# llm-d/llm-d-workload-variant-autoscaler

Hardware: AMD Instinct MI355X
Metric: desired-replica accuracy + SLO-attainment %, Llama-3-8B synthetic QPS ramp (higher is better)
Workload: dtype bf16; 1 GPU; model=meta-llama/Llama-3.1-8B, global_batch=256, seq_len=150, parallelism=dp1, device=AMD Radeon Graphics

## Files before the change

### wva_amd/calibration/model.py

```python
from __future__ import annotations

import math
from dataclasses import dataclass
from typing import List, Optional

import torch

from .. import ops


@dataclass
class LlamaConfig:
    name: str = "llama"
    hidden_size: int = 4096
    intermediate_size: int = 14336
    num_layers: int = 32
    num_q_heads: int = 32
    num_kv_heads: int = 8
    head_dim: int = 128
    vocab_size: int = 128256
    rope_theta: float = 500000.0
    rms_eps: float = 1e-5

    @property
# ... 66 lines not shown
            return torch.empty(rows, cols, device=device, dtype=dtype).normal_(
                0.0, std, generator=gen
            )

        self.input_norm = torch.ones(h, device=device, dtype=dtype)
        self.post_attn_norm = torch.ones(h, device=device, dtype=dtype)
        self.wqkv = w(cfg.q_size + 2 * cfg.kv_size, h)
        self.wo = w(h, cfg.q_size)
        self.w_gate_up = w(2 * cfg.intermediate_size, h)
        self.w_down = w(h, cfg.intermediate_size)


class LlamaDecodeModel:

    def __init__(
        self,
        cfg: LlamaConfig,
        max_batch: int = 256,
        max_seq: int = 2048,
        device: str = "cuda",
        seed: int = 0,
        kv_dtype: str = "bf16",
        weights_dtype: str = "bf16",
    ):
        self.cfg = cfg
        self.device = torch.device(device)
        self.dtype = torch.bfloat16
        if weights_dtype not in ("bf16", "fp8"):
            raise ValueError(f"weights_dtype must be bf16|fp8")
        self.weights_dtype = weights_dtype
        if kv_dtype not in ("bf16", "fp8"):
            raise ValueError(f"kv_dtype must be bf16|fp8, got {kv_dtype}")
        self.kv_dtype = kv_dtype
        self.cache_dtype = (
            torch.float8_e4m3fn if kv_dtype == "fp8" else torch.bfloat16
        )
        self.max_batch = max_batch
        self.max_seq = max_seq
        gen = torch.Generator(device=self.device)
        gen.manual_seed(seed)

        self.embed = torch.empty(
            cfg.vocab_size, cfg.hidden_size, device=self.device, dtype=self.dtype
        ).normal_(0.0, 0.02, generator=gen)
        self.layers: List[_DecoderLayer] = [
            _DecoderLayer(cfg, self.device, self.dtype, gen)
            for _ in range(cfg.num_layers)
        ]
# ... 42 lines not shown
    def _linear(self, x: torch.Tensor, layer, name: str) -> torch.Tensor:
        if self.weights_dtype == "bf16":
            w = getattr(layer, name) if layer is not None else self.lm_head
            return ops.linear(x, w)
        w8, w_scale = (
            getattr(layer, name + "_q") if layer is not None else self.lm_head_q
        )
        if not x.is_cuda:
            return (
                x.float() @ (w8.float() * w_scale[:, None]).t()
            ).to(x.dtype)
        if x.shape[0] <= 64 and x.shape[1] % 128 == 0:
            from .. import ops as _ops

            return _ops._require_ext().skinny_linear_fp8(x, w8, w_scale)
        return (x @ (w8.to(x.dtype) * w_scale[:, None].to(x.dtype)).t())

    @torch.no_grad()
    def decode_step(self, token_ids: torch.Tensor) -> torch.Tensor:
        cfg = self.cfg
        B = token_ids.shape[0]
        positions = self.context_lens[:B].clone()

        ctx = positions + 1
        x = self.embed.index_select(0, token_ids)
        residual: Optional[torch.Tensor] = None

        for li, layer in enumerate(self.layers):
            if residual is None:
                residual = x.clone()
                h = ops.rmsnorm(x, layer.input_norm, None, cfg.rms_eps)
            else:
                h = ops.rmsnorm(x, layer.input_norm, residual, cfg.rms_eps)

            qkv = self._linear(h, layer, "wqkv")
            q = ops.rope_append_kv(
                qkv, self.k_cache[li][:B], self.v_cache[li][:B],
                positions, cfg.num_q_heads, cfg.num_kv_heads, cfg.rope_theta,
            )

            attn = ops.gqa_decode_attn(
                q, self.k_cache[li][:B], self.v_cache[li][:B], ctx, self.scale
            )
            x = self._linear(attn.reshape(B, cfg.q_size), layer, "wo")

            h2 = ops.rmsnorm(x, layer.post_attn_norm, residual, cfg.rms_eps)
            gate_up = self._linear(h2, layer, "w_gate_up")
            act = ops.silu_mul_fused(gate_up)
            x = self._linear(act, layer, "w_down")

        final = ops.rmsnorm(x, self.final_norm, residual, cfg.rms_eps)
        logits = self._linear(final, None, "lm_head")
        self.context_lens[:B] += 1
        return logits

    @torch.no_grad()
    def prefill(self, token_ids: torch.Tensor) -> torch.Tensor:
        cfg = self.cfg
        if self.weights_dtype != "bf16":
            raise NotImplementedError(
                "prefill with fp8 weights is not implemented (the "
                "weight-only fp8 mode targets decode; prefill would "
                "dequantize every layer per pass)"
            )
        B, S = token_ids.shape
        T = B * S
# ... 83 lines not shown
```

### wva_amd/ops/__init__.py

```python
from __future__ import annotations

import glob
import importlib.util
import math
import os
from typing import Optional

import torch

_HERE = os.path.dirname(os.path.abspath(__file__))
_ext = None
_ext_error: Optional[str] = None


def _try_load_extension():
    global _ext, _ext_error
    if _ext is not None:
        return _ext
    candidates = sorted(glob.glob(os.path.join(_HERE, "_wva_ops*.so")))
    if not candidates:
        _ext_error = (
            f"HIP extension _wva_ops*.so not found in {_HERE}; build it with "
            "`python -m wva_amd.ops.build` (or __graft_entry__.build())"
        )
# ... 238 lines not shown
    return silu_mul_ref(gate_up[:, :inter], gate_up[:, inter:]).to(
        gate_up.dtype
    )


def gqa_decode_attn(
    q: torch.Tensor,
    k_cache: torch.Tensor,
    v_cache: torch.Tensor,
    context_lens: torch.Tensor,
    scale: Optional[float] = None,
) -> torch.Tensor:
    if scale is None:
        scale = 1.0 / math.sqrt(q.shape[-1])
    if q.is_cuda:
        return _require_ext().gqa_decode_attn(
            q, k_cache, v_cache, context_lens.to(torch.int32), scale
        )
    return gqa_decode_attn_ref(q, k_cache, v_cache, context_lens, scale).to(
        q.dtype
    )


def moe_route(router_logits: torch.Tensor, top_k: int):
    if router_logits.is_cuda:
        return tuple(
            _require_ext().moe_route(
                router_logits.float().contiguous(), top_k
            )
        )
    return moe_route_ref(router_logits, top_k)


def moe_gate_up_swiglu(
    x: torch.Tensor,
    w_gate_up: torch.Tensor,
    expert_offsets: torch.Tensor,
    sorted_slots: torch.Tensor,
    top_k: int,
) -> torch.Tensor:
    if x.is_cuda:
        return _require_ext().moe_gate_up_swiglu(
            x, w_gate_up, expert_offsets, sorted_slots, top_k
        )
    return moe_gate_up_swiglu_ref(
        x, w_gate_up, expert_offsets, sorted_slots, top_k
# ... 81 lines not shown
```

### wva_amd/ops/csrc/attention.hip

```cpp
#include "common.h"

#include <type_traits>

#define HEAD_DIM 128
#define MAX_G 8
#define TILE 64
#define NUM_WAVES 4
#define ROW_DW 66
#define S_ROW 65

template <bool KV_FP8>
using kv_elem_t = std::conditional_t<KV_FP8, fp8_t, bf16>;

__device__ __forceinline__ long ws_row_offset(int b, int kvh, int g, int split,
                                              int num_kv_heads, int G,
                                              int num_splits) {
  return ((((long)b * num_kv_heads + kvh) * G + g) * num_splits + split) *
         (2 + HEAD_DIM);
}

__device__ __forceinline__ long pack8_fp8(const float* v, float inv_scale) {
  unsigned int lo = 0, hi = 0;
  lo = __builtin_amdgcn_cvt_pk_fp8_f32(v[0] * inv_scale, v[1] * inv_scale,
                                       lo, false);
  lo = __builtin_amdgcn_cvt_pk_fp8_f32(v[2] * inv_scale, v[3] * inv_scale,
                                       lo, true);
  hi = __builtin_amdgcn_cvt_pk_fp8_f32(v[4] * inv_scale, v[5] * inv_scale,
                                       hi, false);
  hi = __builtin_amdgcn_cvt_pk_fp8_f32(v[6] * inv_scale, v[7] * inv_scale,
                                       hi, true);
  return (long)(((unsigned long)hi << 32) | lo);
}

struct QFrags {
  bf16x8_frag bf[4];
  long fp8[4];
  float scale;
};

template <bool KV_FP8>
__device__ __forceinline__ QFrags load_q_frags(const bf16* __restrict__ q,
                                               int b, int kvh, int G,
                                               int num_q_heads, int lane,
                                               int wave, int g, int k0,
                                               float* qmax_lds) {
  QFrags qf;
  qf.scale = 1.0f;
#pragma unroll
  for (int kk = 0; kk < 4; ++kk) qf.fp8[kk] = 0;
  float qv[4][8];
#pragma unroll
  for (int kk = 0; kk < 4; ++kk)
#pragma unroll
    for (int i = 0; i < 8; ++i) qv[kk][i] = 0.0f;
  if (g < G) {
    const bf16* qrow = q + ((long)b * num_q_heads + kvh * G + g) * HEAD_DIM;
#pragma unroll
    for (int kk = 0; kk < 4; ++kk) {
      const short* src = reinterpret_cast<const short*>(qrow + 32 * kk + k0);
#pragma unroll
      for (int i = 0; i < 8; ++i) {
        qf.bf[kk][i] = src[i];
        const bf16 bv = *reinterpret_cast<const bf16*>(&src[i]);
        qv[kk][i] = bf2f(bv);
      }
    }
  } else {
#pragma unroll
    for (int kk = 0; kk < 4; ++kk)
#pragma unroll
      for (int i = 0; i < 8; ++i) qf.bf[kk][i] = 0;
  }
  if constexpr (KV_FP8) {
    float amax = 0.0f;
#pragma unroll
    for (int kk = 0; kk < 4; ++kk)
#pragma unroll
      for (int i = 0; i < 8; ++i) amax = fmaxf(amax, fabsf(qv[kk][i]));
    amax = wave_reduce_max(amax);
    if (lane == 0) qmax_lds[wave] = amax;
    __syncthreads();
    float m0 = qmax_lds[0];
#pragma unroll
    for (int w2 = 1; w2 < NUM_WAVES; ++w2) m0 = fmaxf(m0, qmax_lds[w2]);
    qf.scale = fmaxf(m0 / 448.0f, 1e-12f);
    const float inv = 1.0f / qf.scale;
#pragma unroll
    for (int kk = 0; kk < 4; ++kk) qf.fp8[kk] = pack8_fp8(qv[kk], inv);
    __syncthreads();
  }
  return qf;
}

struct SoftmaxStep {
  float p;
  float corr;
};

__device__ __forceinline__ SoftmaxStep online_softmax_step(
    const float* __restrict__ s_row, int tn, int lane, float& m, float& s) {
  const bool live = lane < tn;
  const float score = live ? s_row[lane] : -INFINITY;
  const float tile_max = wave_reduce_max(score);
  const float m_new = fmaxf(m, tile_max);
  const float p = live ? __expf(score - m_new) : 0.0f;
  const float tile_sum = wave_reduce_sum(p);
  const float corr = (m == -INFINITY) ? 0.0f : __expf(m - m_new);
  s = s * corr + tile_sum;
  m = m_new;
  return {p, corr};
}

template <bool KV_FP8>
__global__ __launch_bounds__(256, 2) void gqa_decode_attn_v4_kernel(
    bf16* __restrict__ out,
    float* __restrict__ workspace,
    const bf16* __restrict__ q,
    const void* __restrict__ k_cache,
    const void* __restrict__ v_cache,
    const int* __restrict__ context_lens,
    const int num_q_heads,
    const int num_kv_heads,
    const int max_seq,
    const float scale) {
  const int b = blockIdx.x;
  const int kvh = blockIdx.y;
  const int split = blockIdx.z;
  const int num_splits = gridDim.z;
  const int G = num_q_heads / num_kv_heads;
  const int ctx = context_lens[b];

  const int lane = threadIdx.x & (WAVE_SIZE - 1);
  const int wave = threadIdx.x / WAVE_SIZE;
  const int frag_col = lane % 16;
  const int frag_k0 = 8 * (lane / 16);

  __shared__ float s_smem[MAX_G][S_ROW];
  __shared__ unsigned int v_smem[TILE * ROW_DW];
  __shared__ float p_smem[MAX_G][TILE];
  float* qmax_lds = nullptr;
  if constexpr (KV_FP8) {
    __shared__ float qmax_smem[NUM_WAVES];
    qmax_lds = qmax_smem;
  }

  const QFrags qf = load_q_frags<KV_FP8>(q, b, kvh, G, num_q_heads, lane,
                                         wave, frag_col, frag_k0, qmax_lds);

  const int heads_mine = (G > wave) ? (G - wave + NUM_WAVES - 1) / NUM_WAVES : 0;
  float m[2], s[2], acc[2][2];
#pragma unroll
  for (int j = 0; j < 2; ++j) {
    m[j] = -INFINITY;
    s[j] = 0.0f;
    acc[j][0] = acc[j][1] = 0.0f;
  }

  const long slab_off = ((long)b * num_kv_heads + kvh) * max_seq * HEAD_DIM;
  const auto* k_slab =
      reinterpret_cast<const kv_elem_t<KV_FP8>*>(k_cache) + slab_off;
  const auto* v_slab =
      reinterpret_cast<const kv_elem_t<KV_FP8>*>(v_cache) + slab_off;

  for (int t0 = split * TILE; t0 < ctx; t0 += num_splits * TILE) {
    const int tn = min(TILE, ctx - t0);

    if constexpr (KV_FP8) {
      const int tile_g8 = tn * (HEAD_DIM / 8);
      const fp8_t* v_src = v_slab + (long)t0 * HEAD_DIM;
      for (int idx = wave * WAVE_SIZE + lane; idx < tile_g8;
// ... 93 lines not shown
  if (num_splits == 1) {
    for (int j = 0; j < heads_mine; ++j) {
      const int g = wave + j * NUM_WAVES;
      const float inv = s[j] > 0.0f ? 1.0f / s[j] : 0.0f;
      bf16x2* orow = reinterpret_cast<bf16x2*>(
          out + ((long)b * num_q_heads + kvh * G + g) * HEAD_DIM);
      orow[lane] = bf16x2{f2bf(acc[j][0] * inv), f2bf(acc[j][1] * inv)};
    }
  } else {
    for (int j = 0; j < heads_mine; ++j) {
      const int g = wave + j * NUM_WAVES;
      float* wsp = workspace +
          ws_row_offset(b, kvh, g, split, num_kv_heads, G, num_splits);
      if (lane == 0) {
        wsp[0] = m[j];
        wsp[1] = s[j];
      }
      wsp[2 + 2 * lane] = acc[j][0];
      wsp[2 + 2 * lane + 1] = acc[j][1];
    }
  }
}

template <bool KV_FP8>
__global__ __launch_bounds__(256, 2) void gqa_decode_attn_v5_kernel(
    bf16* __restrict__ out,
    float* __restrict__ workspace,
    const bf16* __restrict__ q,
    const void* __restrict__ k_cache,
    const void* __restrict__ v_cache,
    const int* __restrict__ context_lens,
    const int num_q_heads,
    const int num_kv_heads,
    const int max_seq,
    const float scale) {
  const int b = blockIdx.x;
  const int kvh = blockIdx.y;
  const int split = blockIdx.z;
  const int num_splits = gridDim.z;
  const int G = num_q_heads / num_kv_heads;
  const int ctx = context_lens[b];

  const int lane = threadIdx.x & (WAVE_SIZE - 1);
  const int wave = threadIdx.x / WAVE_SIZE;
  const int frag_col = lane % 16;
  const int frag_k0 = 8 * (lane / 16);

  __shared__ float s_smem[MAX_G][S_ROW];
  __shared__ unsigned int v_smem[TILE * ROW_DW];
  __shared__ float p_smem[MAX_G][TILE];
  __shared__ float corr_smem[MAX_G];
  __shared__ float sum_smem[MAX_G];
  __shared__ float m_smem[MAX_G];
  float* qmax_lds = nullptr;
  if constexpr (KV_FP8) {
    __shared__ float qmax_smem[NUM_WAVES];
    qmax_lds = qmax_smem;
  }

  const QFrags qf = load_q_frags<KV_FP8>(q, b, kvh, G, num_q_heads, lane,
                                         wave, frag_col, frag_k0, qmax_lds);

  const int heads_mine = (G > wave) ? (G - wave + NUM_WAVES - 1) / NUM_WAVES : 0;
  float m[2], s[2];
#pragma unroll
  for (int j = 0; j < 2; ++j) {
    m[j] = -INFINITY;
    s[j] = 0.0f;
  }
  f32x4_frag acc_pv[2] = {f32x4_frag{0.f, 0.f, 0.f, 0.f},
                          f32x4_frag{0.f, 0.f, 0.f, 0.f}};

  const long slab_off = ((long)b * num_kv_heads + kvh) * max_seq * HEAD_DIM;
  const auto* k_slab =
      reinterpret_cast<const kv_elem_t<KV_FP8>*>(k_cache) + slab_off;
  const auto* v_slab =
      reinterpret_cast<const kv_elem_t<KV_FP8>*>(v_cache) + slab_off;

  for (int t0 = split * TILE; t0 < ctx; t0 += num_splits * TILE) {
    const int tn = min(TILE, ctx - t0);

    if constexpr (KV_FP8) {
      const int tile_g8 = tn * (HEAD_DIM / 8);
      const fp8_t* v_src = v_slab + (long)t0 * HEAD_DIM;
      for (int idx = wave * WAVE_SIZE + lane; idx < tile_g8;
           idx += NUM_WAVES * WAVE_SIZE) {
        const int row = idx >> 4;
        const int d8 = (idx & 15) * 8;
        const unsigned short* src =
            reinterpret_cast<const unsigned short*>(
                v_src + (long)row * HEAD_DIM + d8);
        unsigned int* dst = &v_smem[row * ROW_DW + d8 / 2];
#pragma unroll
        for (int j = 0; j < 4; ++j) {
          const float2_vt f = unpk2_fp8(src[j]);
          const bf16x2 packed{f2bf(f[0]), f2bf(f[1])};
          dst[j] = *reinterpret_cast<const unsigned int*>(&packed);
        }
      }
    } else {
      typedef __attribute__((ext_vector_type(2))) unsigned int uint2_t;
      const int tile_u2 = tn * (HEAD_DIM / 4);
      const unsigned int* v_src =
          reinterpret_cast<const unsigned int*>(v_slab + (long)t0 * HEAD_DIM);
      for (int idx = wave * WAVE_SIZE + lane; idx < tile_u2;
           idx += NUM_WAVES * WAVE_SIZE) {
        const int row = idx >> 5;
        const int d2 = (idx & 31) * 2;
        const uint2_t val = *reinterpret_cast<const uint2_t*>(&v_src[idx * 2]);
        *reinterpret_cast<uint2_t*>(&v_smem[row * ROW_DW + d2]) = val;
      }
    }

    {
      const int prow = 16 * wave + (lane % 16);
      const int pos = t0 + prow;
      const int pos_c = pos < max_seq ? pos : max_seq - 1;
      const int k0 = frag_k0;
      f32x4_frag sf = {0.f, 0.f, 0.f, 0.f};
      if constexpr (KV_FP8) {
        const long* ksrc = reinterpret_cast<const long*>(
            k_slab + (long)pos_c * HEAD_DIM);
        const int l0 = k0 / 8;
#pragma unroll
        for (int kk = 0; kk < 4; ++kk) {
          const long a8 = ksrc[kk * 4 + l0];
          sf = __builtin_amdgcn_mfma_f32_16x16x32_fp8_fp8(
              a8, qf.fp8[kk], sf, 0, 0, 0);
        }
      } else {
#pragma unroll
        for (int kk = 0; kk < 4; ++kk) {
          bf16x8_frag a_frag;
          const short* src = reinterpret_cast<const short*>(
              k_slab + (long)pos_c * HEAD_DIM) + 32 * kk + k0;
#pragma unroll
          for (int i = 0; i < 8; ++i) a_frag[i] = src[i];
          sf = __builtin_amdgcn_mfma_f32_16x16x32_bf16(a_frag, qf.bf[kk],
                                                       sf, 0, 0, 0);
        }
      }
      const float s_eff = KV_FP8 ? scale * qf.scale : scale;
      const int g = lane & 15;
      if (g < G) {
#pragma unroll
        for (int i = 0; i < 4; ++i) {
          const int t = 16 * wave + (lane >> 4) * 4 + i;
          s_smem[g][t] = (t < tn) ? sf[i] * s_eff : -INFINITY;
        }
      }
    }
    __syncthreads();

    for (int j = 0; j < heads_mine; ++j) {
      const int g = wave + j * NUM_WAVES;
      const SoftmaxStep st = online_softmax_step(s_smem[g], tn, lane, m[j], s[j]);
      p_smem[g][lane] = st.p;
      if (lane == 0) corr_smem[g] = st.corr;
    }
    __syncthreads();

    {
      bf16x8_frag p_frag[2];
#pragma unroll
      for (int kk = 0; kk < 2; ++kk) {
        const int g = lane % 16;
        const int pos0 = 32 * kk + 8 * (lane / 16);
        if (g < G) {
#pragma unroll
          for (int i = 0; i < 8; ++i)
            p_frag[kk][i] = f2bf_bits(p_smem[g][pos0 + i]);
        } else {
#pragma unroll
          for (int i = 0; i < 8; ++i) p_frag[kk][i] = 0;
        }
      }
      const unsigned short* v_u16 =
          reinterpret_cast<const unsigned short*>(v_smem);
#pragma unroll
      for (int nsub = 0; nsub < 2; ++nsub) {
        const int dim = 16 * (wave + 4 * nsub) + (lane % 16);
        f32x4_frag d = acc_pv[nsub];
#pragma unroll
        for (int i = 0; i < 4; ++i) {
          const int h = (lane >> 4) * 4 + i;
          d[i] *= (h < G) ? corr_smem[h] : 0.0f;
        }
#pragma unroll
        for (int kk = 0; kk < 2; ++kk) {
          bf16x8_frag v_frag;
          const int pos0 = 32 * kk + 8 * (lane / 16);
#pragma unroll
          for (int i = 0; i < 8; ++i) {
            const int t = pos0 + i;
            v_frag[i] = (t < tn)
                ? (short)v_u16[(t * ROW_DW + (dim >> 1)) * 2 + (dim & 1)]
                : (short)0;
          }
          d = __builtin_amdgcn_mfma_f32_16x16x32_bf16(p_frag[kk], v_frag, d,
                                                      0, 0, 0);
        }
        acc_pv[nsub] = d;
      }
    }
    __syncthreads();
  }

  for (int j = 0; j < heads_mine; ++j) {
    const int g = wave + j * NUM_WAVES;
    if (lane == 0) {
      sum_smem[g] = s[j];
      m_smem[g] = m[j];
    }
  }
  __syncthreads();

  if (num_splits == 1) {
#pragma unroll
    for (int nsub = 0; nsub < 2; ++nsub) {
      const int dim = 16 * (wave + 4 * nsub) + (lane & 15);
#pragma unroll
// ... 101 lines not shown
  if (max_ctx_hint > 0) {
    const int by_work = max_ctx_hint / (min_tiles * TILE);
    if (by_work > cap) cap = by_work;
  }
  if (splits > cap) splits = cap;
  const int max_useful = max_ctx_hint > 0 ? (max_ctx_hint + 2 * TILE - 1) / (2 * TILE) : splits;
  if (splits > max_useful && max_useful >= 1) splits = max_useful;
  return splits < 1 ? 1 : splits;
}

extern "C" void launch_gqa_decode_attn(
    void* out, void* workspace, const void* q, const void* k_cache,
    const void* v_cache, const int* context_lens, int batch, int num_q_heads,
    int num_kv_heads, int max_seq, int num_splits, float scale, int variant,
    int kv_fp8, hipStream_t stream) {
  const auto kernel =
      variant == 5 ? (kv_fp8 ? gqa_decode_attn_v5_kernel<true>
                             : gqa_decode_attn_v5_kernel<false>)
                   : (kv_fp8 ? gqa_decode_attn_v4_kernel<true>
                             : gqa_decode_attn_v4_kernel<false>);
  hipLaunchKernelGGL(kernel, dim3(batch, num_kv_heads, num_splits), dim3(256),
                     0, stream, (bf16*)out, (float*)workspace, (const bf16*)q,
                     k_cache, v_cache, context_lens, num_q_heads, num_kv_heads,
                     max_seq, scale);
  if (num_splits > 1) {
    hipLaunchKernelGGL(gqa_decode_attn_merge_kernel,
                       dim3(batch, num_q_heads), dim3(64 * MERGE_WAVES), 0,
                       stream, (bf16*)out, (const float*)workspace,
                       num_q_heads, num_kv_heads, num_splits);
  }
}
```

### wva_amd/ops/csrc/common.h

```cpp
#pragma once

#include <hip/hip_runtime.h>
#include <hip/hip_bf16.h>

#define WAVE_SIZE 64

using bf16 = __hip_bfloat16;
using bf16x2 = __hip_bfloat162;

__device__ __forceinline__ float bf2f(bf16 v) { return __bfloat162float(v); }
__device__ __forceinline__ bf16 f2bf(float v) { return __float2bfloat16(v); }

typedef __attribute__((ext_vector_type(8))) short bf16x8_frag;
typedef __attribute__((ext_vector_type(4))) float f32x4_frag;
using moe_bf16x8 = bf16x8_frag;
using moe_f32x4 = f32x4_frag;

__device__ __forceinline__ short f2bf_bits(float v) {
  const bf16 b = f2bf(v);
  return *reinterpret_cast<const short*>(&b);
}

__device__ __forceinline__ float wave_reduce_sum(float v) {
#pragma unroll
  for (int offset = 32; offset > 0; offset >>= 1) {
    v += __shfl_xor(v, offset, WAVE_SIZE);
  }
  return v;
}

__device__ __forceinline__ float wave_reduce_max(float v) {
#pragma unroll
  for (int offset = 32; offset > 0; offset >>= 1) {
    v = fmaxf(v, __shfl_xor(v, offset, WAVE_SIZE));
  }
  return v;
}

__device__ __forceinline__ float block_reduce_sum(float v, float* lds) {
  const int lane = threadIdx.x & (WAVE_SIZE - 1);
  const int wave = threadIdx.x / WAVE_SIZE;
  const int num_waves = blockDim.x / WAVE_SIZE;
  v = wave_reduce_sum(v);
// ... 28 lines not shown
```

### wva_amd/ops/csrc/ops.cpp

```cpp

#include <torch/extension.h>
#include <hip/hip_runtime.h>
#include <c10/hip/HIPStream.h>

#include <string>

extern "C" void launch_rmsnorm(void* out, void* residual_out,
                               const void* input, const void* residual,
                               const void* weight, float eps, int rows,
                               int hidden, hipStream_t stream);
extern "C" void launch_rope(void* q, void* k, const int* positions, int tokens,
                            int num_q_heads, int num_k_heads, int head_dim,
                            float theta, hipStream_t stream);
extern "C" void launch_silu_mul(void* out, const void* gate, const void* up,
                                long n, hipStream_t stream);
extern "C" void launch_silu_mul_fused(void* out, const void* gate_up,
                                      long rows, long inter,
                                      hipStream_t stream);
extern "C" void launch_rope_append_kv_fp8(const void* qkv, void* q_out,
                                          void* k_cache, void* v_cache,
                                          const int* positions, int batch,
                                          int num_q_heads, int num_kv_heads,
                                          int head_dim, int max_seq,
                                          float theta, hipStream_t stream);
// ... 9 lines not shown
extern "C" void launch_prefill_attn_ex(void* out, const void* q,
                                       const void* k_cache,
                                       const void* v_cache, int batch,
                                       int seq, int num_q_heads,
                                       int num_kv_heads, int max_seq,
                                       float scale, int kv_fp8,
                                       hipStream_t stream);
extern "C" int skinny_gemm_tile_n(int M);
extern "C" void launch_skinny_gemm(void* c, void* ws, const void* a,
                                   const void* w, int M, int N, int K,
                                   int num_splits, hipStream_t stream);
extern "C" void launch_skinny_gemm_ex(void* c, void* ws, const void* a,
                                      const void* w, const float* w_scale,
                                      int M, int N, int K, int num_splits,
                                      int w_fp8, hipStream_t stream);
extern "C" void launch_gqa_decode_attn(void* out, void* workspace,
                                       const void* q, const void* k_cache,
                                       const void* v_cache,
                                       const int* context_lens, int batch,
                                       int num_q_heads, int num_kv_heads,
                                       int max_seq, int num_splits,
                                       float scale, int variant, int kv_fp8,
                                       hipStream_t stream);

extern "C" int moe_num_m_tiles(int TK, int E);
extern "C" int moe_down_num_splits(int TK, int E, int H, int I);
extern "C" void launch_moe_route(int* topk_idx, float* topk_w,
                                 int* expert_offsets, int* sorted_slots,
                                 const float* logits, int T, int E, int K,
                                 hipStream_t stream);
extern "C" void launch_moe_gate_up_swiglu(void* act, const void* x,
                                          const void* w,
                                          const int* expert_offsets,
                                          const int* sorted_slots, int T,
                                          int E, int top_k, int H, int I,
                                          hipStream_t stream);
extern "C" void launch_moe_down_combine(void* out, float* ws,
                                        const void* act, const void* w,
                                        const float* topk_w,
                                        const int* expert_offsets,
                                        const int* sorted_slots, int T,
                                        int E, int top_k, int H, int I,
                                        int num_splits, hipStream_t stream);

namespace {

// ... 142 lines not shown
  const int G = num_q_heads / num_kv_heads;
  TORCH_CHECK(G <= 8, "GQA group size must be <= 8");
  TORCH_CHECK(v_cache.sizes() == k_cache.sizes(), "k/v cache mismatch");
  auto out = torch::empty_like(q);
  const int num_splits =
      gqa_decode_attn_num_splits(batch, num_kv_heads, max_seq);
  if (variant == AttnVariant::Auto) {
    variant = (G >= 8 || num_splits == 1) ? AttnVariant::V5 : AttnVariant::V4;
  }
  torch::Tensor workspace;
  void* ws_ptr = nullptr;
  if (num_splits > 1) {
    workspace = torch::empty(
        {(long)batch * num_kv_heads * G * num_splits * (2 + head_dim)},
        q.options().dtype(torch::kFloat32));
    ws_ptr = workspace.data_ptr();
  }
  launch_gqa_decode_attn(out.data_ptr(), ws_ptr, q.data_ptr(),
                         k_cache.data_ptr(), v_cache.data_ptr(),
                         context_lens.data_ptr<int>(), batch, num_q_heads,
                         num_kv_heads, max_seq, num_splits, (float)scale,
                         variant == AttnVariant::V5 ? 5 : 4, kv_fp8 ? 1 : 0,
                         current_stream());
  return out;
}

torch::Tensor skinny_linear(torch::Tensor x, torch::Tensor w) {
  check_bf16_contig(x, "x");
  check_bf16_contig(w, "w");
  TORCH_CHECK(x.dim() == 2 && w.dim() == 2, "x [M,K], w [N,K]");
  const int M = x.size(0);
  const int K = x.size(1);
  const int N = w.size(0);
  TORCH_CHECK(w.size(1) == K, "K mismatch");
  TORCH_CHECK(M <= 64, "skinny_linear requires M <= 64");
  TORCH_CHECK(K % 128 == 0, "K must be a multiple of 128");
  auto y = torch::empty({M, N}, x.options());
  const int nt = skinny_gemm_tile_n(M);
  const int sk = skinny_gemm_num_splits(N, K, nt);
  torch::Tensor ws;
  void* ws_ptr = nullptr;
  if (sk > 1) {
    ws = torch::empty({(long)sk * M * N},
                      x.options().dtype(torch::kFloat32));
    ws_ptr = ws.data_ptr();
  }
// ... 177 lines not shown
PYBIND11_MODULE(TORCH_EXTENSION_NAME, m) {
  m.def("rmsnorm", &rmsnorm, "Fused (add-)RMSNorm bf16",
        py::arg("input"), py::arg("weight"), py::arg("residual") = py::none(),
        py::arg("eps") = 1e-5);
  m.def("rope", &rope, "Fused in-place NeoX RoPE on q,k",
        py::arg("q"), py::arg("k"), py::arg("positions"),
        py::arg("theta") = 500000.0);
  m.def("silu_mul", &silu_mul, "Fused SwiGLU silu(gate)*up",
        py::arg("gate"), py::arg("up"));
  m.def("silu_mul_fused", &silu_mul_fused,
        "SwiGLU on the fused [rows, 2*inter] gate_up buffer",
        py::arg("gate_up"));
  m.def("rope_append_kv", &rope_append_kv,
        "RoPE on strided qkv row + KV-cache append; returns contiguous q",
        py::arg("qkv"), py::arg("k_cache"), py::arg("v_cache"),
        py::arg("positions"), py::arg("num_q_heads"), py::arg("num_kv_heads"),
        py::arg("theta") = 500000.0);
  m.def("gqa_decode_attn", &gqa_decode_attn,
        "GQA decode attention over contiguous KV cache; variant pins the "
        "kernel (\"v4\", \"v5\") instead of the measured dispatch (\"auto\")",
        py::arg("q"), py::arg("k_cache"), py::arg("v_cache"),
        py::arg("context_lens"), py::arg("scale"),
        py::arg("variant") = "auto");
  m.def("prefill_attn", &prefill_attn,
        "Causal flash-attention prefill over head-major KV caches",
        py::arg("q"), py::arg("k_cache"), py::arg("v_cache"),
        py::arg("batch"), py::arg("seq"), py::arg("scale"));
  m.def("skinny_linear_fp8", &skinny_linear_fp8,
        "Weight-only fp8 decode GEMM: x[M,K]bf16 @ w[N,K]e4m3^T, M <= 64",
        py::arg("x"), py::arg("w"), py::arg("w_scale"));
  m.def("skinny_linear", &skinny_linear,
        "Weight-streaming decode GEMM: x[M,K] @ w[N,K]^T, M <= 64",
        py::arg("x"), py::arg("w"));
  m.def("moe_route", &moe_route,
        "MoE routing: top-k, softmax weights, expert offsets, sorted slots",
        py::arg("router_logits"), py::arg("top_k"));
  m.def("moe_gate_up_swiglu", &moe_gate_up_swiglu,
        "Grouped gate_up GEMM + SwiGLU over expert-sorted rows",
        py::arg("x"), py::arg("w_gate_up"), py::arg("expert_offsets"),
        py::arg("sorted_slots"), py::arg("top_k"));
  m.def("moe_down_combine", &moe_down_combine,
        "Grouped down GEMM + deterministic top-k combine",
        py::arg("act_sorted"), py::arg("w_down"), py::arg("topk_w"),
        py::arg("expert_offsets"), py::arg("sorted_slots"));
  m.def("moe_down_splits", &moe_down_splits,
        "Split-K factor moe_down_combine uses for these static shapes",
// ... 4 lines not shown
```

### wva_amd/ops/csrc/rope.hip

```cpp

#include "common.h"

__device__ __forceinline__ void rotate_pair(
    const bf16* src, bf16* dst, int d, int half, int head_dim, float pos,
    float theta) {
  const float inv_freq = __powf(theta, -2.0f * (float)d / (float)head_dim);
  const float angle = pos * inv_freq;
  float c, s;
  __sincosf(angle, &s, &c);
  const float x1 = bf2f(src[d]);
  const float x2 = bf2f(src[d + half]);
  dst[d] = f2bf(x1 * c - x2 * s);
  dst[d + half] = f2bf(x2 * c + x1 * s);
}

__global__ void rope_kernel(
    bf16* __restrict__ q,
    bf16* __restrict__ k,
    const int* __restrict__ positions,
    const int num_q_heads,
    const int num_k_heads,
    const int head_dim,
    const float theta) {
  const int token = blockIdx.x;
  const float pos = (float)positions[token];
  const int half = head_dim / 2;
  const int total = (num_q_heads + num_k_heads) * half;

  for (int idx = threadIdx.x; idx < total; idx += blockDim.x) {
    const int head = idx / half;
    const int d = idx % half;
    const bool is_q = head < num_q_heads;
    bf16* base = is_q
        ? q + (long)token * num_q_heads * head_dim + (long)head * head_dim
        : k + (long)token * num_k_heads * head_dim +
              (long)(head - num_q_heads) * head_dim;
// ... 54 lines not shown
    const int* __restrict__ positions,
    const int num_q_heads,
    const int num_kv_heads,
    const int head_dim,
    const int max_seq,
    const float theta) {
  const int b = blockIdx.x;
  const int pos_i = positions[b];
  const float pos = (float)pos_i;
  const int half = head_dim / 2;
  const long qkv_row = (long)b * (num_q_heads + 2 * num_kv_heads) * head_dim;

  const int rot_total = (num_q_heads + num_kv_heads) * half;
  for (int idx = threadIdx.x; idx < rot_total; idx += blockDim.x) {
    const int head = idx / half;
    const int d = idx % half;
    if (head < num_q_heads) {
      const bf16* src = qkv + qkv_row + (long)head * head_dim;
      bf16* dst = q_out + ((long)b * num_q_heads + head) * head_dim;
      rotate_pair(src, dst, d, half, head_dim, pos, theta);
    } else {
      const int kh = head - num_q_heads;
      const bf16* src = qkv + qkv_row + ((long)num_q_heads + kh) * head_dim;
      const float inv_freq =
          __powf(theta, -2.0f * (float)d / (float)head_dim);
      const float angle = pos * inv_freq;
      float c, s;
      __sincosf(angle, &s, &c);
      const float x1 = bf2f(src[d]);
      const float x2 = bf2f(src[d + half]);
      fp8_t* dst = k_cache +
          (((long)b * num_kv_heads + kh) * max_seq + pos_i) * head_dim;
      dst[d] = f2fp8(x1 * c - x2 * s);
      dst[d + half] = f2fp8(x2 * c + x1 * s);
    }
  }
  const int v_total = num_kv_heads * half;
  const bf16x2* vsrc = reinterpret_cast<const bf16x2*>(
      qkv + qkv_row + (long)(num_q_heads + num_kv_heads) * head_dim);
  for (int idx = threadIdx.x; idx < v_total; idx += blockDim.x) {
    const int kh = idx / half;
    const int d2 = idx % half;
    const bf16x2 v2 = vsrc[(long)kh * half + d2];
    unsigned short* dst = reinterpret_cast<unsigned short*>(
        v_cache + (((long)b * num_kv_heads + kh) * max_seq + pos_i) * head_dim);
    dst[d2] = pk2_fp8(bf2f(v2.x), bf2f(v2.y));
  }
}

extern "C" void launch_rope_append_kv_fp8(
    const void* qkv, void* q_out, void* k_cache, void* v_cache,
    const int* positions, int batch, int num_q_heads, int num_kv_heads,
    int head_dim, int max_seq, float theta, hipStream_t stream) {
  dim3 grid(batch);
  dim3 block(256);
  hipLaunchKernelGGL(rope_append_kv_fp8_kernel, grid, block, 0, stream,
                     (const bf16*)qkv, (bf16*)q_out, (fp8_t*)k_cache,
// ... 25 lines not shown
```

Measured before the change: 91.98 %.

## Fuse RoPE and KV-cache append into GQA decode attention kernel

Adds a fused kernel path that applies RoPE to Q and K, appends the new K/V entries to the cache, and runs GQA decode attention in one launch, removing the separate rope_append_kv kernel. It also restructures the v5 kernel's K fragment loading and V tile staging, using an XOR-swizzled LDS layout and batched global loads. The fused path is behind a model flag that defaults to False, so the default decode path is unchanged. The fused path relies on the split that owns the new position writing it before other splits might read it, which risks ordering hazards across blocks.

```diff
diff --git a/wva_amd/calibration/model.py b/wva_amd/calibration/model.py
--- a/wva_amd/calibration/model.py
+++ b/wva_amd/calibration/model.py
@@ -112,8 +112,10 @@
         seed: int = 0,
         kv_dtype: str = "bf16",
         weights_dtype: str = "bf16",
+        fused_rope_attn: bool = False,
     ):
         self.cfg = cfg
+        self.fused_rope_attn = fused_rope_attn
         self.device = torch.device(device)
         self.dtype = torch.bfloat16
         if weights_dtype not in ("bf16", "fp8"):
@@ -202,7 +204,8 @@
         B = token_ids.shape[0]
         positions = self.context_lens[:B].clone()
 
-        ctx = positions + 1
+        if not self.fused_rope_attn:
+            ctx = positions + 1
         x = self.embed.index_select(0, token_ids)
         residual: Optional[torch.Tensor] = None
 
@@ -214,14 +217,22 @@
                 h = ops.rmsnorm(x, layer.input_norm, residual, cfg.rms_eps)
 
             qkv = self._linear(h, layer, "wqkv")
-            q = ops.rope_append_kv(
-                qkv, self.k_cache[li][:B], self.v_cache[li][:B],
-                positions, cfg.num_q_heads, cfg.num_kv_heads, cfg.rope_theta,
-            )
-
-            attn = ops.gqa_decode_attn(
-                q, self.k_cache[li][:B], self.v_cache[li][:B], ctx, self.scale
-            )
+            if self.fused_rope_attn:
+                attn = ops.rope_gqa_decode_attn(
+                    qkv, self.k_cache[li][:B], self.v_cache[li][:B],
+                    positions, cfg.num_q_heads, cfg.num_kv_heads,
+                    cfg.rope_theta, self.scale,
+                )
+            else:
+                q = ops.rope_append_kv(
+                    qkv, self.k_cache[li][:B], self.v_cache[li][:B],
+                    positions, cfg.num_q_heads, cfg.num_kv_heads,
+                    cfg.rope_theta,
+                )
+                attn = ops.gqa_decode_attn(
+                    q, self.k_cache[li][:B], self.v_cache[li][:B], ctx,
+                    self.scale,
+                )
             x = self._linear(attn.reshape(B, cfg.q_size), layer, "wo")
 
             h2 = ops.rmsnorm(x, layer.post_attn_norm, residual, cfg.rms_eps)
diff --git a/wva_amd/ops/__init__.py b/wva_amd/ops/__init__.py
--- a/wva_amd/ops/__init__.py
+++ b/wva_amd/ops/__init__.py
@@ -284,6 +284,30 @@
     )
 
 
+def rope_gqa_decode_attn(
+    qkv: torch.Tensor,
+    k_cache: torch.Tensor,
+    v_cache: torch.Tensor,
+    positions: torch.Tensor,
+    num_q_heads: int,
+    num_kv_heads: int,
+    theta: float,
+    scale: Optional[float] = None,
+    variant: str = "auto",
+) -> torch.Tensor:
+    if scale is None:
+        scale = 1.0 / math.sqrt(k_cache.shape[-1])
+    if qkv.is_cuda:
+        return _require_ext().rope_gqa_decode_attn(
+            qkv, k_cache, v_cache, positions.to(torch.int32),
+            num_q_heads, num_kv_heads, theta, scale, variant,
+        )
+    q = rope_append_kv(
+        qkv, k_cache, v_cache, positions, num_q_heads, num_kv_heads, theta
+    )
+    return gqa_decode_attn(q, k_cache, v_cache, positions + 1, scale)
+
+
 def moe_route(router_logits: torch.Tensor, top_k: int):
     if router_logits.is_cuda:
         return tuple(
diff --git a/wva_amd/ops/csrc/attention.hip b/wva_amd/ops/csrc/attention.hip
--- a/wva_amd/ops/csrc/attention.hip
+++ b/wva_amd/ops/csrc/attention.hip
@@ -38,12 +38,15 @@
   float scale;
 };
 
-template <bool KV_FP8>
+template <bool KV_FP8, bool FUSED_ROPE = false>
 __device__ __forceinline__ QFrags load_q_frags(const bf16* __restrict__ q,
                                                int b, int kvh, int G,
                                                int num_q_heads, int lane,
                                                int wave, int g, int k0,
-                                               float* qmax_lds) {
+                                               float* qmax_lds,
+                                               int num_kv_heads = 0,
+                                               const float* rope_cos = nullptr,
+                                               const float* rope_sin = nullptr) {
   QFrags qf;
   qf.scale = 1.0f;
 #pragma unroll
@@ -53,7 +56,35 @@
   for (int kk = 0; kk < 4; ++kk)
 #pragma unroll
     for (int i = 0; i < 8; ++i) qv[kk][i] = 0.0f;
-  if (g < G) {
+  if constexpr (FUSED_ROPE) {
+    if (g < G) {
+      const bf16* qrow =
+          q + ((long)b * (num_q_heads + 2 * num_kv_heads) + kvh * G + g) *
+                  HEAD_DIM;
+#pragma unroll
+      for (int kk = 0; kk < 2; ++kk) {
+        if (kk == 1) __builtin_amdgcn_sched_barrier(0);
+#pragma unroll
+        for (int i = 0; i < 8; ++i) {
+          const int d = 32 * kk + k0 + i;
+          float y1, y2;
+          rope_apply(bf2f(qrow[d]), bf2f(qrow[d + HEAD_DIM / 2]), rope_cos[d],
+                     rope_sin[d], y1, y2);
+          const bf16 r1 = f2bf(y1);
+          const bf16 r2 = f2bf(y2);
+          qf.bf[kk][i] = *reinterpret_cast<const short*>(&r1);
+          qf.bf[kk + 2][i] = *reinterpret_cast<const short*>(&r2);
+          qv[kk][i] = bf2f(r1);
+          qv[kk + 2][i] = bf2f(r2);
+        }
+      }
+    } else {
+#pragma unroll
+      for (int kk = 0; kk < 4; ++kk)
+#pragma unroll
+        for (int i = 0; i < 8; ++i) qf.bf[kk][i] = 0;
+    }
+  } else if (g < G) {
     const bf16* qrow = q + ((long)b * num_q_heads + kvh * G + g) * HEAD_DIM;
 #pragma unroll
     for (int kk = 0; kk < 4; ++kk) {
@@ -90,6 +121,52 @@
     __syncthreads();
   }
   return qf;
+}
+
+typedef const void* __restrict__ kv_cache_in_ptr;
+template <bool FUSED_ROPE>
+using kv_cache_arg_t = std::conditional_t<FUSED_ROPE, void*, kv_cache_in_ptr>;
+
+template <bool KV_FP8>
+__device__ __forceinline__ void rope_append_prologue(
+    const bf16* __restrict__ qkv, kv_elem_t<KV_FP8>* k_slab,
+    kv_elem_t<KV_FP8>* v_slab, int b, int kvh, int num_q_heads,
+    int num_kv_heads, int pos_i, int max_seq, int split, int num_splits,
+    float theta, int lane, int wave, float* rope_cos, float* rope_sin) {
+  const bool owner = split == (pos_i / TILE) % num_splits && pos_i >= 0 &&
+                     pos_i < max_seq;
+  const bf16* qkv_row =
+      qkv + (long)b * (num_q_heads + 2 * num_kv_heads) * HEAD_DIM;
+  if (wave == 0) {
+    float c, s;
+    rope_sincos(lane, HEAD_DIM, (float)pos_i, theta, c, s);
+    rope_cos[lane] = c;
+    rope_sin[lane] = s;
+    if (owner) {
+      const bf16* src = qkv_row + (long)(num_q_heads + kvh) * HEAD_DIM;
+      float y1, y2;
+      rope_apply(bf2f(src[lane]), bf2f(src[lane + HEAD_DIM / 2]), c, s, y1,
+                 y2);
+      kv_elem_t<KV_FP8>* dst = k_slab + (long)pos_i * HEAD_DIM;
+      if constexpr (KV_FP8) {
+        dst[lane] = f2fp8(y1);
+        dst[lane + HEAD_DIM / 2] = f2fp8(y2);
+      } else {
+        dst[lane] = f2bf(y1);
+        dst[lane + HEAD_DIM / 2] = f2bf(y2);
+      }
+    }
+  } else if (wave == 1 && owner) {
+    const bf16x2 v2 = reinterpret_cast<const bf16x2*>(
+        qkv_row + (long)(num_q_heads + num_kv_heads + kvh) * HEAD_DIM)[lane];
+    if constexpr (KV_FP8) {
+      reinterpret_cast<unsigned short*>(v_slab + (long)pos_i * HEAD_DIM)[lane] =
+          pk2_fp8(bf2f(v2.x), bf2f(v2.y));
+    } else {
+      reinterpret_cast<bf16x2*>(v_slab + (long)pos_i * HEAD_DIM)[lane] = v2;
+    }
+  }
+  __syncthreads();
 }
 
 struct SoftmaxStep {
@@ -111,24 +188,25 @@
   return {p, corr};
 }
 
-template <bool KV_FP8>
+template <bool KV_FP8, bool FUSED_ROPE = false>
 __global__ __launch_bounds__(256, 2) void gqa_decode_attn_v4_kernel(
     bf16* __restrict__ out,
     float* __restrict__ workspace,
     const bf16* __restrict__ q,
-    const void* __restrict__ k_cache,
-    const void* __restrict__ v_cache,
+    kv_cache_arg_t<FUSED_ROPE> k_cache,
+    kv_cache_arg_t<FUSED_ROPE> v_cache,
     const int* __restrict__ context_lens,
     const int num_q_heads,
     const int num_kv_heads,
     const int max_seq,
-    const float scale) {
+    const float scale,
+    const float theta) {
   const int b = blockIdx.x;
   const int kvh = blockIdx.y;
   const int split = blockIdx.z;
   const int num_splits = gridDim.z;
   const int G = num_q_heads / num_kv_heads;
-  const int ctx = context_lens[b];
+  const int ctx = FUSED_ROPE ? context_lens[b] + 1 : context_lens[b];
 
   const int lane = threadIdx.x & (WAVE_SIZE - 1);
   const int wave = threadIdx.x / WAVE_SIZE;
@@ -144,8 +222,23 @@
     qmax_lds = qmax_smem;
   }
 
-  const QFrags qf = load_q_frags<KV_FP8>(q, b, kvh, G, num_q_heads, lane,
-                                         wave, frag_col, frag_k0, qmax_lds);
+  float* rope_cos = nullptr;
+  float* rope_sin = nullptr;
+  if constexpr (FUSED_ROPE) {
+    __shared__ float rope_cs_smem[2][HEAD_DIM / 2];
+    rope_cos = rope_cs_smem[0];
+    rope_sin = rope_cs_smem[1];
+    const long slab = ((long)b * num_kv_heads + kvh) * max_seq * HEAD_DIM;
+    rope_append_prologue<KV_FP8>(
+        q, reinterpret_cast<kv_elem_t<KV_FP8>*>(k_cache) + slab,
+        reinterpret_cast<kv_elem_t<KV_FP8>*>(v_cache) + slab, b, kvh,
+        num_q_heads, num_kv_heads, ctx - 1, max_seq, split, num_splits, theta,
+        lane, wave, rope_cos, rope_sin);
+  }
+
+  const QFrags qf = load_q_frags<KV_FP8, FUSED_ROPE>(
+      q, b, kvh, G, num_q_heads, lane, wave, frag_col, frag_k0, qmax_lds,
+      num_kv_heads, rope_cos, rope_sin);
 
   const int heads_mine = (G > wave) ? (G - wave + NUM_WAVES - 1) / NUM_WAVES : 0;
   float m[2], s[2], acc[2][2];
@@ -285,24 +378,31 @@
   }
 }
 
-template <bool KV_FP8>
+__device__ __forceinline__ int v5_v_off(int row, int ch) {
+  return 256 * row + 16 * (ch ^ (((row & 3) << 2) | ((row >> 2) & 3)));
+}
+typedef __attribute__((ext_vector_type(4))) short v4i16_frag;
+typedef __attribute__((address_space(3))) v4i16_frag* lds_v4i16_ptr;
+
+template <bool KV_FP8, bool FUSED_ROPE = false>
 __global__ __launch_bounds__(256, 2) void gqa_decode_attn_v5_kernel(
     bf16* __restrict__ out,
     float* __restrict__ workspace,
     const bf16* __restrict__ q,
-    const void* __restrict__ k_cache,
-    const void* __restrict__ v_cache,
+    kv_cache_arg_t<FUSED_ROPE> k_cache,
+    kv_cache_arg_t<FUSED_ROPE> v_cache,
     const int* __restrict__ context_lens,
     const int num_q_heads,
     const int num_kv_heads,
     const int max_seq,
-    const float scale) {
+    const float scale,
+    const float theta) {
   const int b = blockIdx.x;
   const int kvh = blockIdx.y;
   const int split = blockIdx.z;
   const int num_splits = gridDim.z;
   const int G = num_q_heads / num_kv_heads;
-  const int ctx = context_lens[b];
+  const int ctx = FUSED_ROPE ? context_lens[b] + 1 : context_lens[b];
 
   const int lane = threadIdx.x & (WAVE_SIZE - 1);
   const int wave = threadIdx.x / WAVE_SIZE;
@@ -310,7 +410,8 @@
   const int frag_k0 = 8 * (lane / 16);
 
   __shared__ float s_smem[MAX_G][S_ROW];
-  __shared__ unsigned int v_smem[TILE * ROW_DW];
+  __shared__ __attribute__((aligned(16))) unsigned int v_smem[TILE * 64];
+  char* v_bytes = reinterpret_cast<char*>(v_smem);
   __shared__ float p_smem[MAX_G][TILE];
   __shared__ float corr_smem[MAX_G];
   __shared__ float sum_smem[MAX_G];
@@ -321,8 +422,23 @@
     qmax_lds = qmax_smem;
   }
 
-  const QFrags qf = load_q_frags<KV_FP8>(q, b, kvh, G, num_q_heads, lane,
-                                         wave, frag_col, frag_k0, qmax_lds);
+  float* rope_cos = nullptr;
+  float* rope_sin = nullptr;
+  if constexpr (FUSED_ROPE) {
+    __shared__ float rope_cs_smem[2][HEAD_DIM / 2];
+    rope_cos = rope_cs_smem[0];
+    rope_sin = rope_cs_smem[1];
+    const long slab = ((long)b * num_kv_heads + kvh) * max_seq * HEAD_DIM;
+    rope_append_prologue<KV_FP8>(
+        q, reinterpret_cast<kv_elem_t<KV_FP8>*>(k_cache) + slab,
+        reinterpret_cast<kv_elem_t<KV_FP8>*>(v_cache) + slab, b, kvh,
+        num_q_heads, num_kv_heads, ctx - 1, max_seq, split, num_splits, theta,
+        lane, wave, rope_cos, rope_sin);
+  }
+
+  const QFrags qf = load_q_frags<KV_FP8, FUSED_ROPE>(
+      q, b, kvh, G, num_q_heads, lane, wave, frag_col, frag_k0, qmax_lds,
+      num_kv_heads, rope_cos, rope_sin);
 
   const int heads_mine = (G > wave) ? (G - wave + NUM_WAVES - 1) / NUM_WAVES : 0;
   float m[2], s[2];
@@ -343,63 +459,88 @@
   for (int t0 = split * TILE; t0 < ctx; t0 += num_splits * TILE) {
     const int tn = min(TILE, ctx - t0);
 
+    const int k_pos = t0 + 16 * wave + (lane % 16);
+    const int k_pos_c = k_pos < max_seq ? k_pos : max_seq - 1;
+    std::conditional_t<KV_FP8, long, bf16x8_frag> k_frag[4];
     if constexpr (KV_FP8) {
-      const int tile_g8 = tn * (HEAD_DIM / 8);
-      const fp8_t* v_src = v_slab + (long)t0 * HEAD_DIM;
-      for (int idx = wave * WAVE_SIZE + lane; idx < tile_g8;
-           idx += NUM_WAVES * WAVE_SIZE) {
-        const int row = idx >> 4;
-        const int d8 = (idx & 15) * 8;
-        const unsigned short* src =
-            reinterpret_cast<const unsigned short*>(
-                v_src + (long)row * HEAD_DIM + d8);
-        unsigned int* dst = &v_smem[row * ROW_DW + d8 / 2];
-#pragma unroll
-        for (int j = 0; j < 4; ++j) {
-          const float2_vt f = unpk2_fp8(src[j]);
-          const bf16x2 packed{f2bf(f[0]), f2bf(f[1])};
-          dst[j] = *reinterpret_cast<const unsigned int*>(&packed);
-        }
-      }
+      const long* ksrc = reinterpret_cast<const long*>(
+          k_slab + (long)k_pos_c * HEAD_DIM);
+#pragma unroll
+      for (int kk = 0; kk < 4; ++kk) k_frag[kk] = ksrc[kk * 4 + frag_k0 / 8];
     } else {
-      typedef __attribute__((ext_vector_type(2))) unsigned int uint2_t;
-      const int tile_u2 = tn * (HEAD_DIM / 4);
-      const unsigned int* v_src =
-          reinterpret_cast<const unsigned int*>(v_slab + (long)t0 * HEAD_DIM);
-      for (int idx = wave * WAVE_SIZE + lane; idx < tile_u2;
-           idx += NUM_WAVES * WAVE_SIZE) {
-        const int row = idx >> 5;
-        const int d2 = (idx & 31) * 2;
-        const uint2_t val = *reinterpret_cast<const uint2_t*>(&v_src[idx * 2]);
-        *reinterpret_cast<uint2_t*>(&v_smem[row * ROW_DW + d2]) = val;
+#pragma unroll
+      for (int kk = 0; kk < 4; ++kk) {
+        const short* src = reinterpret_cast<const short*>(
+            k_slab + (long)k_pos_c * HEAD_DIM) + 32 * kk + frag_k0;
+#pragma unroll
+        for (int i = 0; i < 8; ++i) k_frag[kk][i] = src[i];
       }
     }
 
     {
-      const int prow = 16 * wave + (lane % 16);
-      const int pos = t0 + prow;
-      const int pos_c = pos < max_seq ? pos : max_seq - 1;
-      const int k0 = frag_k0;
+      const int tid = wave * WAVE_SIZE + lane;
+      constexpr int NTHR = NUM_WAVES * WAVE_SIZE;
+      if constexpr (KV_FP8) {
+        typedef __attribute__((ext_vector_type(4))) unsigned int uint4_t;
+        typedef __attribute__((ext_vector_type(4))) unsigned short ushort4_t;
+        constexpr int ITERS = TILE * (HEAD_DIM / 8) / NTHR;
+        const int tile_g8 = tn * (HEAD_DIM / 8);
+        const fp8_t* v_src = v_slab + (long)t0 * HEAD_DIM;
+        ushort4_t raw[ITERS];
+#pragma unroll
+        for (int it = 0; it < ITERS; ++it) {
+          const int idx = tid + it * NTHR;
+          raw[it] = *reinterpret_cast<const ushort4_t*>(
+              v_src + (long)(idx < tile_g8 ? idx : tile_g8 - 1) * 8);
+        }
+#pragma unroll
+        for (int it = 0; it < ITERS; ++it) {
+          const int idx = tid + it * NTHR;
+          const bool live = idx < tile_g8;
+          uint4_t val;
+#pragma unroll
+          for (int j = 0; j < 4; ++j) {
+            const float2_vt f = unpk2_fp8(raw[it][j]);
+            const bf16x2 packed{f2bf(f[0]), f2bf(f[1])};
+            val[j] =
+                live ? *reinterpret_cast<const unsigned int*>(&packed) : 0u;
+          }
+          *reinterpret_cast<uint4_t*>(v_bytes +
+                                      v5_v_off(idx >> 4, idx & 15)) = val;
+        }
+      } else {
+        typedef __attribute__((ext_vector_type(2))) unsigned int uint2_t;
+        constexpr int ITERS = TILE * (HEAD_DIM / 4) / NTHR;
+        const int tile_u2 = tn * (HEAD_DIM / 4);
+        const unsigned int* v_src = reinterpret_cast<const unsigned int*>(
+            v_slab + (long)t0 * HEAD_DIM);
+        uint2_t raw[ITERS];
+#pragma unroll
+        for (int it = 0; it < ITERS; ++it) {
+          const int idx = tid + it * NTHR;
+          raw[it] = *reinterpret_cast<const uint2_t*>(
+              &v_src[(idx < tile_u2 ? idx : tile_u2 - 1) * 2]);
+        }
+#pragma unroll
+        for (int it = 0; it < ITERS; ++it) {
+          const int idx = tid + it * NTHR;
+          const int c8 = idx & 31;
+          *reinterpret_cast<uint2_t*>(v_bytes + v5_v_off(idx >> 5, c8 >> 1) +
+                                      8 * (c8 & 1)) =
+              idx < tile_u2 ? raw[it] : uint2_t{0u, 0u};
+        }
+      }
+    }
+
+    {
       f32x4_frag sf = {0.f, 0.f, 0.f, 0.f};
-      if constexpr (KV_FP8) {
-        const long* ksrc = reinterpret_cast<const long*>(
-            k_slab + (long)pos_c * HEAD_DIM);
-        const int l0 = k0 / 8;
-#pragma unroll
-        for (int kk = 0; kk < 4; ++kk) {
-          const long a8 = ksrc[kk * 4 + l0];
+#pragma unroll
+      for (int kk = 0; kk < 4; ++kk) {
+        if constexpr (KV_FP8) {
           sf = __builtin_amdgcn_mfma_f32_16x16x32_fp8_fp8(
-              a8, qf.fp8[kk], sf, 0, 0, 0);
-        }
-      } else {
-#pragma unroll
-        for (int kk = 0; kk < 4; ++kk) {
-          bf16x8_frag a_frag;
-          const short* src = reinterpret_cast<const short*>(
-              k_slab + (long)pos_c * HEAD_DIM) + 32 * kk + k0;
-#pragma unroll
-          for (int i = 0; i < 8; ++i) a_frag[i] = src[i];
-          sf = __builtin_amdgcn_mfma_f32_16x16x32_bf16(a_frag, qf.bf[kk],
+              k_frag[kk], qf.fp8[kk], sf, 0, 0, 0);
+        } else {
+          sf = __builtin_amdgcn_mfma_f32_16x16x32_bf16(k_frag[kk], qf.bf[kk],
                                                        sf, 0, 0, 0);
         }
       }
@@ -438,8 +579,8 @@
           for (int i = 0; i < 8; ++i) p_frag[kk][i] = 0;
         }
       }
-      const unsigned short* v_u16 =
-          reinterpret_cast<const unsigned short*>(v_smem);
+      const int tr_q = (lane % 16) >> 2;
+      const int tr_p = lane & 3;
 #pragma unroll
       for (int nsub = 0; nsub < 2; ++nsub) {
         const int dim = 16 * (wave + 4 * nsub) + (lane % 16);
@@ -451,15 +592,16 @@
         }
 #pragma unroll
         for (int kk = 0; kk < 2; ++kk) {
-          bf16x8_frag v_frag;
           const int pos0 = 32 * kk + 8 * (lane / 16);
-#pragma unroll
-          for (int i = 0; i < 8; ++i) {
-            const int t = pos0 + i;
-            v_frag[i] = (t < tn)
-                ? (short)v_u16[(t * ROW_DW + (dim >> 1)) * 2 + (dim & 1)]
-                : (short)0;
-          }
+          const int ch = 2 * (wave + 4 * nsub) + (tr_p >> 1);
+          const v4i16_frag lo = __builtin_amdgcn_ds_read_tr16_b64_v4i16(
+              (lds_v4i16_ptr)(v_bytes + v5_v_off(pos0 + tr_q, ch) +
+                              8 * (tr_p & 1)));
+          const v4i16_frag hi = __builtin_amdgcn_ds_read_tr16_b64_v4i16(
+              (lds_v4i16_ptr)(v_bytes + v5_v_off(pos0 + 4 + tr_q, ch) +
+                              8 * (tr_p & 1)));
+          const bf16x8_frag v_frag =
+              __builtin_shufflevector(lo, hi, 0, 1, 2, 3, 4, 5, 6, 7);
           d = __builtin_amdgcn_mfma_f32_16x16x32_bf16(p_frag[kk], v_frag, d,
                                                       0, 0, 0);
         }
@@ -607,7 +749,7 @@
   hipLaunchKernelGGL(kernel, dim3(batch, num_kv_heads, num_splits), dim3(256),
                      0, stream, (bf16*)out, (float*)workspace, (const bf16*)q,
                      k_cache, v_cache, context_lens, num_q_heads, num_kv_heads,
-                     max_seq, scale);
+                     max_seq, scale, 0.0f);
   if (num_splits > 1) {
     hipLaunchKernelGGL(gqa_decode_attn_merge_kernel,
                        dim3(batch, num_q_heads), dim3(64 * MERGE_WAVES), 0,
@@ -615,3 +757,25 @@
                        num_q_heads, num_kv_heads, num_splits);
   }
 }
+
+extern "C" void launch_rope_gqa_decode_attn(
+    void* out, void* workspace, const void* qkv, void* k_cache, void* v_cache,
+    const int* positions, int batch, int num_q_heads, int num_kv_heads,
+    int max_seq, int num_splits, float scale, float theta, int variant,
+    int kv_fp8, hipStream_t stream) {
+  const auto kernel =
+      variant == 5 ? (kv_fp8 ? gqa_decode_attn_v5_kernel<true, true>
+                             : gqa_decode_attn_v5_kernel<false, true>)
+                   : (kv_fp8 ? gqa_decode_attn_v4_kernel<true, true>
+                             : gqa_decode_attn_v4_kernel<false, true>);
+  hipLaunchKernelGGL(kernel, dim3(batch, num_kv_heads, num_splits), dim3(256),
+                     0, stream, (bf16*)out, (float*)workspace,
+                     (const bf16*)qkv, k_cache, v_cache, positions,
+                     num_q_heads, num_kv_heads, max_seq, scale, theta);
+  if (num_splits > 1) {
+    hipLaunchKernelGGL(gqa_decode_attn_merge_kernel,
+                       dim3(batch, num_q_heads), dim3(64 * MERGE_WAVES), 0,
+                       stream, (bf16*)out, (const float*)workspace,
+                       num_q_heads, num_kv_heads, num_splits);
+  }
+}
diff --git a/wva_amd/ops/csrc/common.h b/wva_amd/ops/csrc/common.h
--- a/wva_amd/ops/csrc/common.h
+++ b/wva_amd/ops/csrc/common.h
@@ -19,6 +19,45 @@
 __device__ __forceinline__ short f2bf_bits(float v) {
   const bf16 b = f2bf(v);
   return *reinterpret_cast<const short*>(&b);
+}
+
+struct RopeCosSin {
+  float c, s;
+};
+
+static __device__ __noinline__ RopeCosSin rope_cos_sin(float freq_exp, float pos,
+                                                float theta) {
+  const float inv_freq = __powf(theta, freq_exp);
+  const float angle = pos * inv_freq;
+  RopeCosSin r;
+  __sincosf(angle, &r.s, &r.c);
+  return r;
+}
+
+__device__ __forceinline__ void rope_sincos(int d, int head_dim, float pos,
+                                            float theta, float& c, float& s) {
+  const RopeCosSin r =
+      rope_cos_sin(-2.0f * (float)d / (float)head_dim, pos, theta);
+  c = r.c;
+  s = r.s;
+}
+
+__device__ __forceinline__ void rope_apply(float x1, float x2, float c,
+                                           float s, float& y1, float& y2) {
+  float t1, t2;
+  asm("v_mul_f32 %0, %1, %2" : "=v"(t1) : "v"(x2), "v"(s));
+  asm("v_fma_f32 %0, %1, %2, -%3" : "=v"(y1) : "v"(x1), "v"(c), "v"(t1));
+  asm("v_mul_f32 %0, %1, %2" : "=v"(t2) : "v"(x2), "v"(c));
+  asm("v_fma_f32 %0, %1, %2, %3" : "=v"(y2) : "v"(x1), "v"(s), "v"(t2));
+}
+
+__device__ __forceinline__ void rope_rotate_pair(float x1, float x2, int d,
+                                                 int head_dim, float pos,
+                                                 float theta, float& y1,
+                                                 float& y2) {
+  float c, s;
+  rope_sincos(d, head_dim, pos, theta, c, s);
+  rope_apply(x1, x2, c, s, y1, y2);
 }
 
 __device__ __forceinline__ float wave_reduce_sum(float v) {
diff --git a/wva_amd/ops/csrc/ops.cpp b/wva_amd/ops/csrc/ops.cpp
--- a/wva_amd/ops/csrc/ops.cpp
+++ b/wva_amd/ops/csrc/ops.cpp
@@ -55,6 +55,11 @@
                                        int max_seq, int num_splits,
                                        float scale, int variant, int kv_fp8,
                                        hipStream_t stream);
+extern "C" void launch_rope_gqa_decode_attn(
+    void* out, void* workspace, const void* qkv, void* k_cache, void* v_cache,
+    const int* positions, int batch, int num_q_heads, int num_kv_heads,
+    int max_seq, int num_splits, float scale, float theta, int variant,
+    int kv_fp8, hipStream_t stream);
 
 extern "C" int moe_num_m_tiles(int TK, int E);
 extern "C" int moe_down_num_splits(int TK, int E, int H, int I);
@@ -243,6 +248,58 @@
                          num_kv_heads, max_seq, num_splits, (float)scale,
                          variant == AttnVariant::V5 ? 5 : 4, kv_fp8 ? 1 : 0,
                          current_stream());
+  return out;
+}
+
+torch::Tensor rope_gqa_decode_attn(torch::Tensor qkv, torch::Tensor k_cache,
+                                   torch::Tensor v_cache,
+                                   torch::Tensor positions,
+                                   int64_t num_q_heads, int64_t num_kv_heads,
+                                   double theta, double scale,
+                                   const std::string& variant_name) {
+  AttnVariant variant = parse_attn_variant(variant_name);
+  check_bf16_contig(qkv, "qkv");
+  const bool kv_fp8 = check_cache_contig(k_cache, "k_cache");
+  TORCH_CHECK(check_cache_contig(v_cache, "v_cache") == kv_fp8,
+              "k/v cache dtype mismatch");
+  TORCH_CHECK(positions.is_cuda() && positions.scalar_type() == torch::kInt32,
+              "positions must be int32 on GPU");
+  TORCH_CHECK(qkv.dim() == 2, "qkv must be [B, (Hq+2Hk)*D]");
+  TORCH_CHECK(k_cache.dim() == 4,
+              "k_cache must be [B, Hk, S, D] (head-major)");
+  const int batch = qkv.size(0);
+  const int head_dim = k_cache.size(3);
+  const int max_seq = k_cache.size(2);
+  TORCH_CHECK(head_dim == 128, "head_dim must be 128 (Llama-3 family)");
+  TORCH_CHECK(num_kv_heads >= 1 && num_q_heads % num_kv_heads == 0,
+              "Hq must divide by Hk");
+  const int G = num_q_heads / num_kv_heads;
+  TORCH_CHECK(G <= 8, "GQA group size must be <= 8");
+  TORCH_CHECK(k_cache.size(0) >= batch, "cache batch smaller than qkv's");
+  TORCH_CHECK(positions.numel() >= batch, "positions shorter than batch");
+  TORCH_CHECK(k_cache.size(1) == num_kv_heads, "Hk mismatch");
+  TORCH_CHECK(v_cache.sizes() == k_cache.sizes(), "k/v cache mismatch");
+  TORCH_CHECK(qkv.size(1) == (num_q_heads + 2 * num_kv_heads) * head_dim,
+              "qkv width mismatch");
+  auto out = torch::empty({batch, num_q_heads, head_dim}, qkv.options());
+  const int num_splits =
+      gqa_decode_attn_num_splits(batch, (int)num_kv_heads, max_seq);
+  if (variant == AttnVariant::Auto) {
+    variant = (G >= 8 || num_splits == 1) ? AttnVariant::V5 : AttnVariant::V4;
+  }
+  torch::Tensor workspace;
+  void* ws_ptr = nullptr;
+  if (num_splits > 1) {
+    workspace = torch::empty(
+        {(long)batch * num_kv_heads * G * num_splits * (2 + head_dim)},
+        qkv.options().dtype(torch::kFloat32));
+    ws_ptr = workspace.data_ptr();
+  }
+  launch_rope_gqa_decode_attn(
+      out.data_ptr(), ws_ptr, qkv.data_ptr(), k_cache.data_ptr(),
+      v_cache.data_ptr(), positions.data_ptr<int>(), batch, (int)num_q_heads,
+      (int)num_kv_heads, max_seq, num_splits, (float)scale, (float)theta,
+      variant == AttnVariant::V5 ? 5 : 4, kv_fp8 ? 1 : 0, current_stream());
   return out;
 }
 
@@ -466,6 +523,12 @@
         py::arg("q"), py::arg("k_cache"), py::arg("v_cache"),
         py::arg("context_lens"), py::arg("scale"),
         py::arg("variant") = "auto");
+  m.def("rope_gqa_decode_attn", &rope_gqa_decode_attn,
+        "RoPE + KV-cache append + GQA decode attention in one launch; "
+        "attends over positions + 1 entries",
+        py::arg("qkv"), py::arg("k_cache"), py::arg("v_cache"),
+        py::arg("positions"), py::arg("num_q_heads"), py::arg("num_kv_heads"),
+        py::arg("theta"), py::arg("scale"), py::arg("variant") = "auto");
   m.def("prefill_attn", &prefill_attn,
         "Causal flash-attention prefill over head-major KV caches",
         py::arg("q"), py::arg("k_cache"), py::arg("v_cache"),
diff --git a/wva_amd/ops/csrc/rope.hip b/wva_amd/ops/csrc/rope.hip
--- a/wva_amd/ops/csrc/rope.hip
+++ b/wva_amd/ops/csrc/rope.hip
@@ -4,14 +4,11 @@
 __device__ __forceinline__ void rotate_pair(
     const bf16* src, bf16* dst, int d, int half, int head_dim, float pos,
     float theta) {
-  const float inv_freq = __powf(theta, -2.0f * (float)d / (float)head_dim);
-  const float angle = pos * inv_freq;
-  float c, s;
-  __sincosf(angle, &s, &c);
-  const float x1 = bf2f(src[d]);
-  const float x2 = bf2f(src[d + half]);
-  dst[d] = f2bf(x1 * c - x2 * s);
-  dst[d + half] = f2bf(x2 * c + x1 * s);
+  float y1, y2;
+  rope_rotate_pair(bf2f(src[d]), bf2f(src[d + half]), d, head_dim, pos, theta,
+                   y1, y2);
+  dst[d] = f2bf(y1);
+  dst[d + half] = f2bf(y2);
 }
 
 __global__ void rope_kernel(
@@ -112,17 +109,13 @@
     } else {
       const int kh = head - num_q_heads;
       const bf16* src = qkv + qkv_row + ((long)num_q_heads + kh) * head_dim;
-      const float inv_freq =
-          __powf(theta, -2.0f * (float)d / (float)head_dim);
-      const float angle = pos * inv_freq;
-      float c, s;
-      __sincosf(angle, &s, &c);
-      const float x1 = bf2f(src[d]);
-      const float x2 = bf2f(src[d + half]);
+      float y1, y2;
+      rope_rotate_pair(bf2f(src[d]), bf2f(src[d + half]), d, head_dim, pos,
+                       theta, y1, y2);
       fp8_t* dst = k_cache +
           (((long)b * num_kv_heads + kh) * max_seq + pos_i) * head_dim;
-      dst[d] = f2fp8(x1 * c - x2 * s);
-      dst[d + half] = f2fp8(x2 * c + x1 * s);
+      dst[d] = f2fp8(y1);
+      dst[d + half] = f2fp8(y2);
     }
   }
   const int v_total = num_kv_heads * half;
```

Result: slower. 77.35 % (-15.9%).
